# AIM-Harvard/pyradiomics

Measured on AMD Instinct MI355X. Metric: Mvoxels/s for GLCM+GLRLM build, 512^3 vol @32 bins, higher is better.
Workload: dtype u8 levels / u32 counts / f64 out; 1 GPU; GLCM+GLRLM matrix build, 512^3 int32+uint8 volume resident in HBM, 32 grey levels, full mask, 13 angles, uniform levels; one volume per GPU (batch sharding, no collective); size=512, levels=32, dist=uniform, deferred_mode=pipeline

## Files before the change

pyradiomics_amd/csrc/kernels_sweepfw.h:

```cpp
#pragma once
#include "kernels_sweep.h"

namespace prad {

enum FwPhase { FP_INIT, FP_GRAB, FP_CTRL, FP_ISSUE, FP_WAIT_ROWS, FP_WAIT_PACK, FP_GROUP, FP_PACK, FP_SLOW, FP_FLUSH, FP_DRAIN,
               FP_TOTAL, FP_REALTIME, FP_NGROUP, FP_NGROUP_PACK, FP_NSLOW, FP_COUNT };
#ifdef PRAD_FW_STAMPS
__device__ unsigned long long prad_fw_stamps[2 * 8192 * FP_COUNT];
struct FwClock {
  unsigned long long last, first, rt0;
  unsigned acc[FP_COUNT];
  __device__ __forceinline__ void start() {
#pragma unroll
    for (int i = 0; i < FP_COUNT; i++) acc[i] = 0;
    rt0 = __builtin_amdgcn_s_memrealtime();
    first = last = __builtin_readcyclecounter();
  }
  template <int PH>
  __device__ __forceinline__ void lap() {
    const unsigned long long now = __builtin_readcyclecounter();
    acc[PH] += (unsigned)(now - last);
    last = now;
  }
  template <int PH>
// ... 711 lines not shown
              t += U;
              row += U * du;
              off += (long long)U * delta;
              ri += (long long)U * dri;
              zpos += U;
            };
            for (int gi = 0; gi < ng; gi++) {
              load_group(va, off);
              one_group(va, gi == 0);
            }
            if (du != 0 && (row < 0 || row >= NU)) wrap = true;
            continue;
          }
        }
        u32 c[KW];
        if (closing) {
#pragma unroll
          for (int w = 0; w < KW; w++) c[w] = 0;
        } else {
          load_row(lp + off, c);
        }
        clk.template lap<FP_CTRL>();
        single_step(c, tail);
        clk.template lap<FP_SLOW>();
        clk.template count<FP_NSLOW>();
        safe = 0;
        young = 0;
        if (closing) {
          if (finish) break;
          reset_lines(0);
          row -= du * NU;
          off -= (long long)du * NU * D.sU;
          ri -= (long long)du * NU * sUr;
          zpos = 65;
          wrap = false;
          continue;
        }
        t++;
        zpos++;
        row += du;
        off += delta;
        ri += dri;
        if (du != 0 && (row < 0 || row >= NU)) wrap = true;
      }
    }
  }
};

template <bool ZA>
__device__ __forceinline__ void fw_row_word(const FwTab &T, u32 one, int &s, u32 c, u32 x) {
  int t;
#define PRAD_FW_RCOL(J)                                                                                          \
  "v_cmpx_ne_u32_sdwa vcc, %[c], %[x] src0_sel:BYTE_" #J " src1_sel:BYTE_" #J "\n\t"                             \
  "v_add_u32_sdwa %[t], %[s], %[c] dst_sel:DWORD dst_unused:UNUSED_PAD src0_sel:DWORD src1_sel:BYTE_" #J "\n\t"   \
  "v_mul_u32_u24_sdwa %[s], %[P4], %[c] dst_sel:DWORD dst_unused:UNUSED_PAD src0_sel:DWORD src1_sel:BYTE_" #J "\n\t" \
  "v_cmpx_ne_u32_sdwa vcc, %[x], %[z] src0_sel:BYTE_" #J " src1_sel:DWORD\n\t"                                  \
  "ds_add_u32 %[t], %[one]\n\t"                                                                                  \
  "s_mov_b64 exec, -1\n\t"                                                                                       \
  "v_add_u32 %[s], %[Q], %[s]\n\t"
#define PRAD_FW_RCOL_NZ(J)                                                                                       \
  "v_cmpx_ne_u32_sdwa vcc, %[c], %[x] src0_sel:BYTE_" #J " src1_sel:BYTE_" #J "\n\t"                             \
  "v_add_u32_sdwa %[t], %[s], %[c] dst_sel:DWORD dst_unused:UNUSED_PAD src0_sel:DWORD src1_sel:BYTE_" #J "\n\t"   \
  "ds_add_u32 %[t], %[one]\n\t"                                                                                  \
  "v_mul_u32_u24_sdwa %[s], %[P4], %[c] dst_sel:DWORD dst_unused:UNUSED_PAD src0_sel:DWORD src1_sel:BYTE_" #J "\n\t" \
  "s_mov_b64 exec, -1\n\t"                                                                                       \
  "v_add_u32 %[s], %[Q], %[s]\n\t"
  if (ZA) {
    u32 z = 0;
    asm volatile("" : "+v"(z));
    asm volatile(PRAD_FW_RCOL(0) PRAD_FW_RCOL(1) PRAD_FW_RCOL(2) PRAD_FW_RCOL(3)
                 : [s] "+v"(s), [t] "=&v"(t)
                 : [c] "v"(c), [x] "v"(x), [one] "v"(one), [P4] "s"(T.P4), [Q] "s"(T.Q), [z] "v"(z)
                 : "vcc", "memory");
  } else {
    asm volatile(PRAD_FW_RCOL_NZ(0) PRAD_FW_RCOL_NZ(1) PRAD_FW_RCOL_NZ(2) PRAD_FW_RCOL_NZ(3)
                 : [s] "+v"(s), [t] "=&v"(t)
                 : [c] "v"(c), [x] "v"(x), [one] "v"(one), [P4] "s"(T.P4), [Q] "s"(T.Q)
                 : "vcc", "memory");
  }
#undef PRAD_FW_RCOL
#undef PRAD_FW_RCOL_NZ
}

template <bool LONG, bool ZA>
__device__ __forceinline__ void fw_rows_role(const HistLayout &h, const FwTab &T, u32 *lds, const uint8_t *__restrict__ L,
                                             long long nrows, int NX, int pitch, int bx, int nblocks) {
  const int lane = threadIdx.x & 63, wave = threadIdx.x >> 6, wpb = blockDim.x >> 6;
  const int dummy = T.dummy0b + 4 * lane;
  u32 one = 1;
  asm volatile("" : "+v"(one));
  uint8_t *tile = reinterpret_cast<uint8_t *>(lds) + ((fw_lds_bytes(h) + 15) & ~(size_t)15) + (size_t)wave * 64 * PRAD_ROW_PITCH;
  const int RSTEP = nrows >= 4096 ? 8 : 1;
  const long long ngroups = RSTEP == 8 ? ((nrows + 511) / 512) * 8 : (nrows + 63) / 64;
  const long long nwaves = (long long)nblocks * wpb;
  const bool vec16 = (pitch & 15) == 0 && ((uintptr_t)L & 15) == 0;
  for (long long grp = (long long)bx * wpb + wave; grp < ngroups; grp += nwaves) {
    const long long r0 = RSTEP == 8 ? (grp >> 3) * 512 + (grp & 7) : grp * 64;
    int s = 0;
    u32 pw = 0;
    uint4 nx4[4];
    auto fetch = [&](int xc) __attribute__((always_inline)) {
#pragma unroll
      for (int j = 0; j < 4; j++) {
        const int rr = j * 16 + (lane >> 2);
        const int cx = xc + (lane & 3) * 16;
        uint4 q = make_uint4(0, 0, 0, 0);
        if (r0 + RSTEP * rr < nrows && cx < NX) {
          q = *reinterpret_cast<const uint4 *>(L + (r0 + RSTEP * rr) * pitch + cx);
          const int valid = NX - cx;
          if (valid < 16) {
            u32 *qw = reinterpret_cast<u32 *>(&q);
#pragma unroll
            for (int wd = 0; wd < 4; wd++) {
              const int keep = valid - 4 * wd;
              qw[wd] = keep >= 4 ? qw[wd] : (keep <= 0 ? 0u : (qw[wd] & ((1u << (8 * keep)) - 1u)));
            }
          }
        }
        nx4[j] = q;
      }
    };
    if (vec16) fetch(0);
    for (int xc = 0; xc < NX; xc += 64) {
      if (vec16) {
#pragma unroll
        for (int j = 0; j < 4; j++) *reinterpret_cast<uint4 *>(tile + (j * 16 + (lane >> 2)) * PRAD_ROW_PITCH + (lane & 3) * 16) = nx4[j];
        __builtin_amdgcn_wave_barrier();
        if (xc + 64 < NX) fetch(xc + 64);
      } else {
        const bool xin = xc + lane < NX;
#pragma unroll 8
        for (int rr = 0; rr < 64; rr++) {
          uint8_t b = 0;
          if (xin && r0 + RSTEP * rr < nrows) b = L[(r0 + RSTEP * rr) * pitch + xc + lane];
          tile[rr * PRAD_ROW_PITCH + lane] = b;
        }
      }
      __builtin_amdgcn_wave_barrier();
      const uint4 *row = reinterpret_cast<const uint4 *>(tile + lane * PRAD_ROW_PITCH);
#pragma unroll
      for (int q = 0; q < 4; q++) {
        const uint4 d = row[q];
        const u32 wds[4] = {d.x, d.y, d.z, d.w};
        const unsigned m = (pw >> 24) ? (unsigned)(s - __mul24((int)(pw >> 24), T.P4)) : 0u;
        if (LONG && __ballot(m + 16 * T.Q > (unsigned)T.lenlim) != 0) {
#pragma unroll 1
          for (int k = 0; k < 4; k++) {
            const u32 c = wds[k], x = __builtin_amdgcn_alignbyte(c, pw, 3);
            const unsigned m4 = (pw >> 24) ? (unsigned)(s - __mul24((int)(pw >> 24), T.P4)) : 0u;
            if (__ballot(m4 + 4 * T.Q > (unsigned)T.lenlim) != 0) {
#pragma unroll
              for (int b = 0; b < 4; b++) fw_checked<LONG>(T, dummy, s, (int)((x >> (8 * b)) & 0xffu), (int)((c >> (8 * b)) & 0xffu), false);
            } else {
              fw_row_word<ZA>(T, one, s, c, x);
            }
            pw = c;
          }
        } else {
#pragma unroll
          for (int k = 0; k < 4; k++) {
            fw_row_word<ZA>(T, one, s, wds[k], __builtin_amdgcn_alignbyte(wds[k], pw, 3));
            pw = wds[k];
          }
        }
      }
      __builtin_amdgcn_wave_barrier();
    }
    fw_checked<LONG>(T, dummy, s, (int)(pw >> 24), 0, false);
  }
}

template <bool LONG>
__global__ void __launch_bounds__(1024) sweep_fw_rows_kernel(const uint8_t *__restrict__ L, long long nrows, int NX, int pitch,
                                                            int slot, int Ng, int Nr, int RS, u32 *__restrict__ glcm_acc,
                                                            u32 *__restrict__ glrlm_acc, int *__restrict__ flags) {
  extern __shared__ u32 lds[];
  if (flags[0]) return;
  const HistLayout h = hist_layout(true, true, true, Ng, RS);
  if ((unsigned)(size_t)((lds_u32 *)lds) != 0u) {
    if (threadIdx.x == 0) atomicExch(flags + 2, 1);
    return;
  }
  for (int i = threadIdx.x; i < h.words + Ng + 1; i += blockDim.x) lds[i] = 0;
  __syncthreads();
  FwTab T;
  T.init(h, Nr, glrlm_acc + (size_t)slot * Ng * Nr);
  if (flags[3] != 0) fw_rows_role<LONG, true>(h, T, lds, L, nrows, NX, pitch, (int)blockIdx.x, (int)gridDim.x);
  else fw_rows_role<LONG, false>(h, T, lds, L, nrows, NX, pitch, (int)blockIdx.x, (int)gridDim.x);
  flush_block_hist<true, true, true>(lds + Ng + 1, h, Nr, slot, glcm_acc, glrlm_acc);
}

template <bool LONG, int K, bool HASPAD, bool PACK>
__global__ void __launch_bounds__(1024) sweep_fw_kernel(FwSet set, PackJob pj, const uint8_t *__restrict__ L,
                                                        const uint8_t *__restrict__ rowzero, int Ng, int Nr, int RS,
                                                        u32 *__restrict__ glcm_acc, u32 *__restrict__ glrlm_acc,
                                                        int *__restrict__ work, int *__restrict__ flags) {
  extern __shared__ u32 lds[];
  int role = 0;
  while (role + 1 < set.count && (int)blockIdx.x >= set.first_block[role + 1]) role++;
  const int bx = (int)blockIdx.x - set.first_block[role], nblocks = set.first_block[role + 1] - set.first_block[role];
  const int wpb = (int)(blockDim.x >> 6);
  const long long pw = __builtin_amdgcn_readfirstlane((int)(blockIdx.x * wpb + (threadIdx.x >> 6)));
  PackWave pk(pj, pw, (long long)gridDim.x * wpb);
  FwClock clk;
  clk.start();
#ifdef PRAD_FW_SETPRIO
  __builtin_amdgcn_s_setprio(PRAD_FW_SETPRIO);
#endif
  if (flags[0] == 0) {
    const bool anyzero = flags[3] != 0;
    const HistLayout h = hist_layout(true, true, true, Ng, RS);
    if ((unsigned)(size_t)((lds_u32 *)lds) != 0u) {
      if (threadIdx.x == 0) atomicExch(flags + 2, 1);
    } else {
      for (int i = threadIdx.x; i < h.words + Ng + 1; i += blockDim.x) lds[i] = 0;
      __syncthreads();
      clk.lap<FP_INIT>();
      const FwDesc &D = set.d[role];
      FwTab T;
      T.init(h, Nr, glrlm_acc + (size_t)D.slot * Ng * Nr);
      int *wk = work + PRAD_FW_WORK_STRIDE * PRAD_FW_DOMAINS * role;
      if (D.dx == 0) {
        FwWave<LONG, K, 0, HASPAD, PACK> w(T, set.NX);
        w.run(D, set.NX, set.pitch, set.nrows, L, rowzero, anyzero, wk, bx, nblocks, pk, pj, set.xcd != 0, clk);
      } else if (D.dx > 0) {
        FwWave<LONG, K, 1, HASPAD, PACK> w(T, set.NX);
        w.run(D, set.NX, set.pitch, set.nrows, L, rowzero, anyzero, wk, bx, nblocks, pk, pj, set.xcd != 0, clk);
      } else {
        FwWave<LONG, K, -1, HASPAD, PACK> w(T, set.NX);
        w.run(D, set.NX, set.pitch, set.nrows, L, rowzero, anyzero, wk, bx, nblocks, pk, pj, set.xcd != 0, clk);
      }
      clk.lap<FP_CTRL>();
      flush_block_hist<true, true, true>(lds + Ng + 1, h, Nr, D.slot, glcm_acc, glrlm_acc);
      clk.lap<FP_FLUSH>();
    }
  }
  if (PACK) pk.drain(pj);
  clk.lap<FP_DRAIN>();
  clk.store(PACK ? 1 : 0);
}

}
```

pyradiomics_amd/csrc/prad_api.hip:

```cpp
#include "prad_runtime.h"
#include "kernels_generic.h"
#include "kernels_pairs.h"
#include "kernels_sweep.h"
#include "kernels_sweepfw.h"
#include "kernels_sweepfw2.h"
#include "kernels_neigh.h"
#include "kernels_glszm.h"
#include "kernels_voxel.h"
#include "kernels_voxslide.h"
#include "kernels_mcc.h"
#include "kernels_voxtex.h"
#include "kernels_binning.h"

#include <algorithm>
#include <atomic>
#include <chrono>
#include <cmath>
#include <condition_variable>
#include <cstdlib>
#include <deque>
#include <limits>
#include <mutex>
#include <thread>

// ... 140 lines not shown

int generic_glcm(Call &k, int Ng, double *out) {
  const size_t per = (size_t)Ng * Ng * k.Na;
  PRAD_HIP(hipMemsetAsync(out, 0, sizeof(double) * per * k.vm.nvox, k.s));
  const long long threads = (long long)k.vm.nvox * k.vm.boxmax;
  PRAD_TRY(check_grid(threads, "GLCM"));
  Timed t(*k.c, "generic", k.s);
  hipLaunchKernelGGL(gen_glcm_kernel, dim3(blocks_for(threads)), dim3(256), 0, k.s, k.g, k.vm, k.image, k.mask,
                     k.angles_d, k.Na, Ng, out, k.flags_d + 1);
  return check_launch("gen_glcm_kernel");
}

int generic_glrlm(Call &k, int Ng, int Nr, double *out) {
  const size_t per = (size_t)Ng * Nr * k.Na;
  PRAD_HIP(hipMemsetAsync(out, 0, sizeof(double) * per * k.vm.nvox, k.s));
  int *multi = nullptr;
  PRAD_TRY(k.c->get<int>("multi", (size_t)k.vm.nvox * k.Na, &multi));
  PRAD_HIP(hipMemsetAsync(multi, 0, sizeof(int) * k.vm.nvox * k.Na, k.s));
  const long long threads = (long long)k.vm.nvox * k.vm.boxmax * k.Na;
  PRAD_TRY(check_grid(threads, "GLRLM"));
  Timed t(*k.c, "generic", k.s);
  hipLaunchKernelGGL(gen_glrlm_kernel, dim3(blocks_for(threads)), dim3(256), 0, k.s, k.g, k.vm, k.image, k.mask,
                     k.angles_d, k.Na, Ng, Nr, out, multi, k.flags_d + 1);
  PRAD_TRY(check_launch("gen_glrlm_kernel"));
  const long long pthreads = (long long)k.vm.nvox * Ng * k.Na;
  hipLaunchKernelGGL(glrlm_prune_kernel, dim3(blocks_for(pthreads)), dim3(256), 0, k.s, out, multi, k.vm.nvox, Ng,
                     Nr, k.Na);
  return check_launch("glrlm_prune_kernel");
}

int generic_gldm(Call &k, int Ng, int alpha, double *out) {
  const size_t per = (size_t)Ng * (2 * (size_t)k.Na + 1);
  PRAD_HIP(hipMemsetAsync(out, 0, sizeof(double) * per * k.vm.nvox, k.s));
  const long long threads = (long long)k.vm.nvox * k.vm.boxmax;
  PRAD_TRY(check_grid(threads, "GLDM"));
  Timed t(*k.c, "generic", k.s);
  hipLaunchKernelGGL(gen_gldm_kernel, dim3(blocks_for(threads)), dim3(256), 0, k.s, k.g, k.vm, k.image, k.mask,
                     k.angles_d, k.Na, Ng, alpha, out, k.flags_d + 1);
  return check_launch("gen_gldm_kernel");
}

int generic_ngtdm(Call &k, int Ng, double *out) {
  Timed t(*k.c, "generic", k.s);
  if (k.vm.voxels) {
    hipLaunchKernelGGL(gen_ngtdm_voxel_kernel, dim3(blocks_for(k.vm.nvox, 64)), dim3(64), 0, k.s, k.g, k.vm,
                       k.image, k.mask, k.angles_d, k.Na, Ng, out, k.flags_d + 1);
    return check_launch("gen_ngtdm_voxel_kernel");
  }
  unsigned long long *acc = nullptr;
  const size_t nacc = (size_t)Ng * (k.Na + 1);
  PRAD_TRY(k.c->get<unsigned long long>("ngtdm_acc", nacc, &acc));
  PRAD_HIP(hipMemsetAsync(acc, 0, sizeof(unsigned long long) * nacc, k.s));
  PRAD_TRY(check_grid(k.g.n, "NGTDM"));
  hipLaunchKernelGGL(gen_ngtdm_segment_kernel, dim3(blocks_for(k.g.n)), dim3(256), 0, k.s, k.g, k.vm, k.image,
                     k.mask, k.angles_d, k.Na, Ng, acc, k.flags_d + 1);
  PRAD_TRY(check_launch("gen_ngtdm_segment_kernel"));
  hipLaunchKernelGGL(ngtdm_finalize_kernel, dim3(blocks_for(Ng, 64)), dim3(64), 0, k.s, acc, Ng, k.Na, out);
  return check_launch("ngtdm_finalize_kernel");
}

struct SweepPlan {
  bool ok = false;
  int Nz = 1, Ny = 1, Nx = 1;
  SweepSet lines;
  int row_slot = -1;
  bool skip1 = false;
  bool fused = false;
  int LPL = 1;
  int pitch = 0, padw = 0;
  bool vec_rows = false;
  AngleSet aset;
  int RS = 0;
  bool LONG = false;
  int threads = 256;
  size_t lds_bytes = 0;
  int RSr = 0;
  bool LONGr = false;
  size_t lds_bytes_rows = 0;
  bool fw = false;
  int fwK = 8;
  int fw_blocks = 1;
  int fw_threads = 1024;
  int fw_rows_threads = 512;
  int RSfw = 0;
  bool LONGfw = false;
  size_t lds_fw = 0;
  int RSfw_rows = 0;
  size_t lds_fw_rows = 0;
  bool fw2 = false;
  int RS2 = 0;
  int fw2_copies = 1;
  bool LONGfw2 = false;
  size_t lds_fw2 = 0;
  int pitch16 = 0;
  bool fw2_rows = false;
  int RS2r = 0, fw2r_copies = 1, fw2r_waves = 16;
  bool LONGfw2r = false;
  size_t lds_fw2_rows = 0;
  FwSet fwset;
};

constexpr size_t kHistBudget = 72 * 1024;
constexpr size_t kHistBudgetRows = 36 * 1024;
constexpr int kRowsThreads = 512;
constexpr size_t kHistBudgetFw = 146 * 1024;

int cu_count() {
  static thread_local int cus = 0;
  if (!cus) {
    int dev = 0;
    if (hipGetDevice(&dev) != hipSuccess ||
        hipDeviceGetAttribute(&cus, hipDeviceAttributeMultiprocessorCount, dev) != hipSuccess || cus <= 0)
      cus = 256;
  }
  return cus;
}

int fit_rs(bool glcm, bool glrlm, bool fused, int Ng, int Nr, size_t budget) {
  int lo = 0, hi = Nr;
  if (sizeof(u32) * (size_t)hist_layout(glcm, glrlm, fused, Ng, 1).words > budget) return -1;
  lo = 1;
  while (lo < hi) {
    const int mid = (lo + hi + 1) / 2;
    if (sizeof(u32) * (size_t)hist_layout(glcm, glrlm, fused, Ng, mid).words <= budget) lo = mid;
    else hi = mid - 1;
  }
  return lo;
}

SweepPlan plan_sweep(const Call &k, int Ng, int Nr, bool want_glcm, bool want_glrlm) {
  SweepPlan p;
  if (k.vm.voxels || k.g.nd > 3 || Ng < 1 || Ng > 255 || k.Na > PRAD_MAX_SWEEP) return p;
  int dims[3] = {1, 1, 1};
  for (int d = 0; d < k.g.nd; d++) dims[3 - k.g.nd + d] = k.g.size[d];
  p.Nz = dims[0]; p.Ny = dims[1]; p.Nx = dims[2];
  const int longest = std::max(dims[0], std::max(dims[1], dims[2]));
  if (want_glrlm && Nr < longest) return p;
  if (!want_glrlm) Nr = 1;
  if (want_glcm && want_glrlm) {
    const int rs = fit_rs(true, true, true, Ng, Nr, kHistBudget);
    const int rsr = fit_rs(true, true, true, Ng, Nr, kHistBudgetRows);
    if (Ng <= (255 >> PRAD_FUSED_SHIFT) && rs >= std::min(Nr, 8) && rsr >= std::min(Nr, 4)) {
      p.fused = true;
      p.RS = rs;
      p.RSr = rsr;
    }
  }
  const bool force_fw2 = getenv("PRAD_FORCE_FW2") != nullptr && Ng >= 8;
  if (force_fw2 && want_glcm && want_glrlm && p.Nx > 64 && p.Nx <= 512) p.fused = false;
  if (want_glcm && want_glrlm && !p.fused && (Ng >= 40 || force_fw2) && p.Nx > 64 && p.Nx <= 512 && !getenv("PRAD_NO_FW2")) {
    const long long maxwords = (158 * 1024) / 4;
    const long long room = maxwords / (Ng + 1) - (Ng + 1);
    int copies = 1;
    long long rs2 = std::min<long long>(room, Nr);
    for (int cc = 8; cc >= 2; cc >>= 1)
      if (room / cc >= std::min<long long>(32, Nr)) {
        copies = cc;
        rs2 = std::min<long long>(std::min<long long>(room / cc, 64), Nr);
        break;
      }
    if (const char *e = getenv("PRAD_FW2_COPIES")) {
      copies = std::max(1, std::min(8, atoi(e)));
      rs2 = std::min<long long>(std::min<long long>(room / copies, copies > 1 ? 64 : Nr), Nr);
    }
    if (const char *e = getenv("PRAD_FW2_RS")) rs2 = std::min<long long>(rs2, atoll(e));
    if (rs2 < Nr && ((Ng + 1 + copies * rs2) & 1) == 0) rs2--;
// ... 46 lines not shown
  if (const char *e = getenv("PRAD_THREADS")) {
    const int v = atoi(e);
    if (v == 256 || v == 512 || v == 1024) p.threads = v;
  }
  const size_t hw = (size_t)hist_layout(want_glcm, want_glrlm, p.fused, Ng, p.RSr).words;
  p.lds_bytes_rows = sizeof(u32) * ((hw + 3) & ~(size_t)3) + (kRowsThreads / 64) * 64 * PRAD_ROW_PITCH;
  {
    const double waves = std::max(1.0, (double)(cu_count() / std::max(1, std::min(k.Na, 12))) * 16.0);
    const double cost[3] = {1.0, 0.575, 0.33};
    const int cand[3] = {4, 2, 1};
    double best = 1e300;
    p.LPL = 1;
    for (int i = 0; i < 3; i++) {
      if (cand[i] > 1 && p.Nx < 48 * cand[i]) continue;
      const double chunks = (double)std::max(p.Ny, 1) * ((p.Nx + 64 * cand[i] - 1) / (64 * cand[i]));
      const double t = (chunks <= waves ? 1.0 : chunks / waves + 0.5) * cost[i];
      if (t < best) {
        best = t;
        p.LPL = cand[i];
      }
    }
  }
  if (const char *e = getenv("PRAD_LPL")) {
    const int v = atoi(e);
    if (v == 1 || v == 2 || v == 4) p.LPL = v;
  }
  p.vec_rows = (p.Nx % 16) == 0;
  p.fw = p.fused && p.Nx > 64 && p.Nx <= 1024 && !getenv("PRAD_NO_FW");
  if (p.Nx > 512 && getenv("PRAD_NO_FW16")) p.fw = false;
  if (const char *e = getenv("PRAD_FW_MINVOX")) p.fw = p.fw && k.g.n >= atoll(e);
  p.fwK = p.Nx <= 256 ? 4 : (p.Nx <= 512 ? 8 : 16);
  if (p.fw2) p.fwK = p.Nx <= 256 ? 4 : 8;
  p.padw = (p.fw || p.fw2) ? 0 : std::min(64 * p.LPL, p.Nx);
  p.pitch16 = 2 * ((p.Nx + 7) & ~7);
  p.pitch = (p.Nx + p.padw + 15) & ~15;
  p.lines.count = 0;
  p.aset.count = k.Na;
  for (int a = 0; a < k.Na; a++) {
    int o[3] = {0, 0, 0};
    for (int d = 0; d < k.g.nd; d++) o[3 - k.g.nd + d] = k.angles_h[a * k.g.nd + d];
    int first = 0;
    for (int d = 0; d < 3; d++) {
      if (o[d] < -1 || o[d] > 1) return p;
      if (!first && o[d]) first = o[d];
      p.aset.off[a][d] = o[d];
    }
    if (first != 1) return p;
    if (o[0] == 0 && o[1] == 0) {
      if (p.row_slot >= 0) return p;
      p.row_slot = a;
      continue;
    }
    SweepDesc &D = p.lines.d[p.lines.count++];
    D.slot = a;
    D.NX = p.Nx;
    D.dx = o[2];
    if (o[0] == 1) {
      D.NM = p.Nz; D.NU = p.Ny; D.du = o[1];
      D.sM = (long long)p.Ny * p.pitch; D.sU = p.pitch;
    } else {
      D.NM = p.Ny; D.NU = p.Nz; D.du = 0;
      D.sM = p.pitch; D.sU = (long long)p.Ny * p.pitch;
    }
    D.LXc = (p.Nx + 64 * p.LPL - 1) / (64 * p.LPL);
    D.chunks = (long long)D.NU * D.LXc;
  }
  if ((p.fw || p.fw2) && p.lines.count > 0) {
    size_t budget = kHistBudgetFw;
    if (const char *e = getenv("PRAD_FW_BUDGET_KB")) budget = (size_t)std::max(8, atoi(e)) * 1024;
    p.RSfw = fit_rs(true, true, true, Ng, Nr, budget);
    if (p.RSfw < Nr) {
      for (int rs = p.RSfw; rs >= std::max(16, p.RSfw - 12); rs--) {
        const int d = (((rs + 1) * (Ng + 1)) % 32 + 1) % 32, dist = std::min(d, 32 - d);
        if ((d & 1) && dist >= 5 && dist <= 11) {
          p.RSfw = rs;
          break;
        }
      }
    }
    if (const char *e = getenv("PRAD_FW_RS")) p.RSfw = std::max(1, std::min(p.RSfw, atoi(e)));
    p.LONGfw = p.RSfw < Nr;
    p.lds_fw = fw_lds_bytes(hist_layout(true, true, true, Ng, p.RSfw));
    if (p.row_slot >= 0 && p.fw) {
      if (const char *e = getenv("PRAD_FW_ROWS_THREADS")) p.fw_rows_threads = std::max(64, std::min(1024, atoi(e) & ~63));
      const size_t tiles = (size_t)(p.fw_rows_threads / 64) * 64 * PRAD_ROW_PITCH;
      int rs = fit_rs(true, true, true, Ng, Nr, std::min<size_t>(100 * 1024, (size_t)160 * 1024 - 2048 - tiles));
      for (int r = rs; rs < Nr && r >= std::max(16, rs - 12); r--) {
        const int d = (((r + 1) * (Ng + 1)) % 32 + 1) % 32, dist = std::min(d, 32 - d);
        if ((d & 1) && dist >= 5 && dist <= 11) { rs = r; break; }
      }
      p.RSfw_rows = rs;
      p.lds_fw_rows = ((fw_lds_bytes(hist_layout(true, true, true, Ng, rs)) + 15) & ~(size_t)15) + tiles;
    }
    {
      const int nroles = p.lines.count;
      int total = cu_count();
      if (const char *e = getenv("PRAD_FW_BLOCKS")) total = std::max(nroles, atoi(e));
      if (const char *e = getenv("PRAD_FW_THREADS")) p.fw_threads = std::max(64, std::min(1024, atoi(e) & ~63));
      int bonus[PRAD_MAX_SWEEP] = {0};
      {
        int left = total % nroles;
        const bool as_listed = getenv("PRAD_FW_EXTRA_FIRST") != nullptr;
        for (int cls = as_listed ? 0 : 2; cls >= 0 && left > 0; cls--)
          for (int r = 0; r < nroles && left > 0; r++) {
            const SweepDesc &S = p.lines.d[r];
            const int c = (S.dx != 0 ? 1 : 0) + (S.du != 0 ? 1 : 0);
            if ((as_listed || c == cls) && !bonus[r]) {
              bonus[r] = 1;
              left--;
            }
          }
      }
      p.fwset.first_block[0] = 0;
      for (int r = 0; r < nroles; r++) p.fwset.first_block[r + 1] = p.fwset.first_block[r] + total / nroles + bonus[r];
      for (int r = nroles + 1; r < PRAD_MAX_SWEEP + 1; r++) p.fwset.first_block[r] = p.fwset.first_block[nroles];
      p.fw_blocks = p.fwset.first_block[nroles];
    }
    int per_wave = 6;
    if (const char *e = getenv("PRAD_FW_PER_WAVE")) per_wave = std::max(1, atoi(e));
    p.fwset.count = p.lines.count;
    p.fwset.NX = p.Nx;
    p.fwset.xcd = 0;
    if (const char *e = getenv("PRAD_FW_XCD")) p.fwset.xcd = ((p.fw || p.fw2) && p.Nz >= 64 && atoi(e) != 0) ? 1 : 0;
    for (int i = 0; i < p.lines.count; i++) {
      const SweepDesc &S = p.lines.d[i];
      FwDesc &D = p.fwset.d[i];
      D.slot = S.slot; D.NM = S.NM; D.NU = S.NU; D.du = S.du; D.dx = S.dx; D.sM = S.sM; D.sU = S.sU;
      p.fwset.pitch = p.pitch;
      if (p.fw2) {
        const bool march_z = S.sM >= S.sU;
        D.sM = march_z ? (long long)p.Ny * p.pitch16 : p.pitch16;
        D.sU = march_z ? p.pitch16 : (long long)p.Ny * p.pitch16;
        p.fwset.pitch = p.pitch16;
      }
      p.fwset.nrows = p.Nz * p.Ny;
      const long long want = (long long)per_wave * (p.fwset.first_block[i + 1] - p.fwset.first_block[i]) * (p.fw_threads / 64);
      int pieces = (int)std::max<long long>(1, (want + D.NU - 1) / D.NU);
      int CL = ((D.NM + pieces - 1) / pieces + 7) & ~7;
      CL = std::max(CL, D.NM >= 128 ? 64 : 16);
      const bool march_z_role = S.sM >= S.sU && p.Nz > 1;
      D.dom_kind = march_z_role ? 0 : 1;
      if (p.fwset.xcd && march_z_role) CL = std::max(32, ((D.NM + PRAD_FW_DOMAINS - 1) / PRAD_FW_DOMAINS + 7) & ~7);
      if (const char *e = getenv("PRAD_FW_CL")) CL = std::max(8, atoi(e) & ~7);
      D.CL = CL;
      D.pieces = (D.NM + CL - 1) / CL;
      const long long chunks = (long long)D.NU * D.pieces;
      if (chunks > 2000000000LL) return p;
      D.chunks = (int)chunks;
    }
  } else {
    p.fw = false;
    if (p.fw2) return SweepPlan();
  }
  if (p.row_slot < 0) p.skip1 = false;
  p.ok = true;
  return p;
}

template <bool G, bool R, bool LNG, bool F, int LPL>
int launch_lines_lpl(Call &k, const SweepPlan &p, const uint8_t *levels, int Ng, int Nr, u32 *glcm_acc,
                     u32 *glrlm_acc, int *multi) {
  long long maxchunks = 0;
  for (int i = 0; i < p.lines.count; i++) maxchunks = std::max(maxchunks, p.lines.d[i].chunks);
  const int wpb = p.threads / 64;
  const long long blocks_avail = std::max<long long>(1, (long long)cu_count() / p.lines.count);
  unsigned gx = (unsigned)std::max<long long>(1, std::min<long long>(blocks_avail, (maxchunks + wpb - 1) / wpb));
  if (const char *e = getenv("PRAD_LINES_BLOCKS")) {
    const int v = atoi(e);
// ... 4 lines not shown
  hipLaunchKernelGGL((sweep_lines_kernel<G, R, LNG, F, LPL>), dim3(gx, p.lines.count), dim3(p.threads), p.lds_bytes,
                     k.s, p.lines, levels, Ng, Nr, p.RS, glcm_acc, glrlm_acc, multi, multi + PRAD_MAX_SWEEP,
                     k.flags_d);
  return check_launch("sweep_lines_kernel");
}

template <bool G, bool R, bool LNG, bool F>
int launch_lines(Call &k, const SweepPlan &p, const uint8_t *levels, int Ng, int Nr, u32 *glcm_acc, u32 *glrlm_acc,
                 int *multi) {
  if (p.LPL == 4) return launch_lines_lpl<G, R, LNG, F, 4>(k, p, levels, Ng, Nr, glcm_acc, glrlm_acc, multi);
  if (p.LPL == 2) return launch_lines_lpl<G, R, LNG, F, 2>(k, p, levels, Ng, Nr, glcm_acc, glrlm_acc, multi);
  return launch_lines_lpl<G, R, LNG, F, 1>(k, p, levels, Ng, Nr, glcm_acc, glrlm_acc, multi);
}

template <bool LNG, int K, bool HASPAD, bool PACK>
int launch_fw_kpp(Call &k, const SweepPlan &p, const PackJob &pj, const uint8_t *levels, const uint8_t *rowzero, int Ng, int Nr,
                  u32 *glcm_acc, u32 *glrlm_acc, int *multi, int *flags_d) {
  PRAD_HIP(hipFuncSetAttribute(reinterpret_cast<const void *>(&sweep_fw_kernel<LNG, K, HASPAD, PACK>),
                               hipFuncAttributeMaxDynamicSharedMemorySize, (int)p.lds_fw));
  hipLaunchKernelGGL((sweep_fw_kernel<LNG, K, HASPAD, PACK>), dim3(p.fw_blocks), dim3(p.fw_threads), p.lds_fw, k.s, p.fwset, pj,
                     levels, rowzero, Ng, Nr, p.RSfw, glcm_acc, glrlm_acc, multi + 2 * PRAD_MAX_SWEEP + PRAD_FW_WORK_STRIDE, flags_d);
  return check_launch("sweep_fw_kernel");
}
template <bool LNG, int K, bool HASPAD>
int launch_fw_kp(Call &k, const SweepPlan &p, const PackJob &pj, const uint8_t *levels, const uint8_t *rowzero, int Ng, int Nr,
                 u32 *glcm_acc, u32 *glrlm_acc, int *multi, int *flags_d) {
  if (pj.n16 > 0) return launch_fw_kpp<LNG, K, HASPAD, true>(k, p, pj, levels, rowzero, Ng, Nr, glcm_acc, glrlm_acc, multi, flags_d);
  return launch_fw_kpp<LNG, K, HASPAD, false>(k, p, pj, levels, rowzero, Ng, Nr, glcm_acc, glrlm_acc, multi, flags_d);
}
template <bool LNG, int K>
int launch_fw_k(Call &k, const SweepPlan &p, const PackJob &pj, const uint8_t *levels, const uint8_t *rowzero, int Ng, int Nr,
                u32 *glcm_acc, u32 *glrlm_acc, int *multi, int *flags_d) {
  if (p.Nx != 64 * K) return launch_fw_kp<LNG, K, true>(k, p, pj, levels, rowzero, Ng, Nr, glcm_acc, glrlm_acc, multi, flags_d);
  return launch_fw_kp<LNG, K, false>(k, p, pj, levels, rowzero, Ng, Nr, glcm_acc, glrlm_acc, multi, flags_d);
}
int launch_fw(Call &k, const SweepPlan &p, const PackJob &pj, const uint8_t *levels, const uint8_t *rowzero, int Ng, int Nr,
              u32 *glcm_acc, u32 *glrlm_acc, int *multi, int *flags_d) {
  if (p.fwK == 16)
    return p.LONGfw ? launch_fw_k<true, 16>(k, p, pj, levels, rowzero, Ng, Nr, glcm_acc, glrlm_acc, multi, flags_d)
                    : launch_fw_k<false, 16>(k, p, pj, levels, rowzero, Ng, Nr, glcm_acc, glrlm_acc, multi, flags_d);
  if (p.LONGfw) return p.fwK == 4 ? launch_fw_k<true, 4>(k, p, pj, levels, rowzero, Ng, Nr, glcm_acc, glrlm_acc, multi, flags_d)
                                : launch_fw_k<true, 8>(k, p, pj, levels, rowzero, Ng, Nr, glcm_acc, glrlm_acc, multi, flags_d);
  return p.fwK == 4 ? launch_fw_k<false, 4>(k, p, pj, levels, rowzero, Ng, Nr, glcm_acc, glrlm_acc, multi, flags_d)
                    : launch_fw_k<false, 8>(k, p, pj, levels, rowzero, Ng, Nr, glcm_acc, glrlm_acc, multi, flags_d);
}

template <bool LNG, int K, bool HASPAD, bool SKIP1, bool PACK>
int launch_fw2_khsp(Call &k, const SweepPlan &p, const PackJob &pj, const uint8_t *levels16, int Ng, int Nr, u32 *glcm_acc, u32 *glrlm_acc,
                    int *work, int *flags_d) {
  PRAD_HIP(hipFuncSetAttribute(reinterpret_cast<const void *>(&sweep_fw2_kernel<LNG, K, HASPAD, SKIP1, PACK>),
                               hipFuncAttributeMaxDynamicSharedMemorySize, (int)p.lds_fw2));
  hipLaunchKernelGGL((sweep_fw2_kernel<LNG, K, HASPAD, SKIP1, PACK>), dim3(p.fw_blocks), dim3(1024), p.lds_fw2, k.s, p.fwset, pj, levels16,
                     Ng, Nr, p.RS2, p.fw2_copies, glcm_acc, glrlm_acc, work, flags_d);
  return check_launch("sweep_fw2_kernel");
}
template <bool LNG, int K, bool HASPAD, bool SKIP1>
int launch_fw2_khs(Call &k, const SweepPlan &p, const PackJob &pj, const uint8_t *levels16, int Ng, int Nr, u32 *glcm_acc, u32 *glrlm_acc,
                   int *work, int *flags_d) {
  if (pj.n16 > 0) return launch_fw2_khsp<LNG, K, HASPAD, SKIP1, true>(k, p, pj, levels16, Ng, Nr, glcm_acc, glrlm_acc, work, flags_d);
  return launch_fw2_khsp<LNG, K, HASPAD, SKIP1, false>(k, p, pj, levels16, Ng, Nr, glcm_acc, glrlm_acc, work, flags_d);
}
template <bool LNG, int K>
int launch_fw2_k(Call &k, const SweepPlan &p, const PackJob &pj, const uint8_t *levels16, int Ng, int Nr, u32 *glcm_acc, u32 *glrlm_acc,
                 int *multi, int *flags_d) {
  int *work = multi + 2 * PRAD_MAX_SWEEP + PRAD_FW_WORK_STRIDE;
  if (p.Nx != 64 * K)
    return p.skip1 ? launch_fw2_khs<LNG, K, true, true>(k, p, pj, levels16, Ng, Nr, glcm_acc, glrlm_acc, work, flags_d)
                   : launch_fw2_khs<LNG, K, true, false>(k, p, pj, levels16, Ng, Nr, glcm_acc, glrlm_acc, work, flags_d);
  return p.skip1 ? launch_fw2_khs<LNG, K, false, true>(k, p, pj, levels16, Ng, Nr, glcm_acc, glrlm_acc, work, flags_d)
                 : launch_fw2_khs<LNG, K, false, false>(k, p, pj, levels16, Ng, Nr, glcm_acc, glrlm_acc, work, flags_d);
}
int launch_fw2(Call &k, const SweepPlan &p, const PackJob &pj, const uint8_t *levels16, int Ng, int Nr, u32 *glcm_acc, u32 *glrlm_acc,
               int *multi, int *flags_d) {
  if (p.LONGfw2) return p.fwK == 4 ? launch_fw2_k<true, 4>(k, p, pj, levels16, Ng, Nr, glcm_acc, glrlm_acc, multi, flags_d)
                                 : launch_fw2_k<true, 8>(k, p, pj, levels16, Ng, Nr, glcm_acc, glrlm_acc, multi, flags_d);
  return p.fwK == 4 ? launch_fw2_k<false, 4>(k, p, pj, levels16, Ng, Nr, glcm_acc, glrlm_acc, multi, flags_d)
                    : launch_fw2_k<false, 8>(k, p, pj, levels16, Ng, Nr, glcm_acc, glrlm_acc, multi, flags_d);
}

template <bool LNG>
int launch_fw_rows(Call &k, const SweepPlan &p, const uint8_t *levels, int Ng, int Nr, u32 *glcm_acc, u32 *glrlm_acc, int *flags_d) {
  const long long nrows = (long long)p.Nz * p.Ny, groups = nrows >= 4096 ? ((nrows + 511) / 512) * 8 : (nrows + 63) / 64;
  const int wpb = p.fw_rows_threads / 64;
  const unsigned gx = (unsigned)std::max<long long>(1, std::min<long long>((groups + wpb - 1) / wpb, (long long)cu_count()));
  PRAD_HIP(hipFuncSetAttribute(reinterpret_cast<const void *>(&sweep_fw_rows_kernel<LNG>),
                               hipFuncAttributeMaxDynamicSharedMemorySize, (int)p.lds_fw_rows));
  hipLaunchKernelGGL((sweep_fw_rows_kernel<LNG>), dim3(gx), dim3(p.fw_rows_threads), p.lds_fw_rows, k.s, levels, nrows, p.Nx,
                     p.pitch, p.row_slot, Ng, Nr, p.RSfw_rows, glcm_acc, glrlm_acc, flags_d);
  return check_launch("sweep_fw_rows_kernel");
}

template <bool LNG>
int launch_fw2_rows(Call &k, const SweepPlan &p, const uint8_t *levels16, int Ng, int Nr, u32 *glcm_acc, u32 *glrlm_acc, int *flags_d) {
  const long long nrows = (long long)p.Nz * p.Ny, groups = nrows >= 4096 ? ((nrows + 511) / 512) * 8 : (nrows + 63) / 64;
  const int wpb = p.fw2r_waves;
  const unsigned gx = (unsigned)std::max<long long>(1, std::min<long long>((groups + wpb - 1) / wpb, (long long)cu_count()));
  PRAD_HIP(hipFuncSetAttribute(reinterpret_cast<const void *>(&sweep_fw2_rows_kernel<LNG>),
                               hipFuncAttributeMaxDynamicSharedMemorySize, (int)p.lds_fw2_rows));
  hipLaunchKernelGGL((sweep_fw2_rows_kernel<LNG>), dim3(gx), dim3(64 * wpb), p.lds_fw2_rows, k.s, levels16, nrows, p.Nx, p.pitch16,
                     p.row_slot, Ng, Nr, p.RS2r, p.fw2r_copies, glcm_acc, glrlm_acc, flags_d);
  return check_launch("sweep_fw2_rows_kernel");
}

template <bool G, bool R, bool LNG, bool F>
int launch_rows(Call &k, const SweepPlan &p, const uint8_t *levels, int Ng, int Nr, u32 *glcm_acc, u32 *glrlm_acc,
                int *multi) {
  const long long nrows = (long long)p.Nz * p.Ny;
  const long long groups = (nrows + 63) / 64;
  const int wpb = kRowsThreads / 64;
  const int per_cu = std::max(1, std::min(2048 / kRowsThreads, (int)(160 * 1024 / p.lds_bytes_rows)));
  const unsigned gx = (unsigned)std::max<long long>(1, std::min<long long>((groups + wpb - 1) / wpb, (long long)cu_count() * per_cu));
  PRAD_HIP(hipFuncSetAttribute(reinterpret_cast<const void *>(&sweep_rows_kernel<G, R, LNG, F>),
                               hipFuncAttributeMaxDynamicSharedMemorySize, (int)p.lds_bytes_rows));
  hipLaunchKernelGGL((sweep_rows_kernel<G, R, LNG, F>), dim3(gx), dim3(kRowsThreads), p.lds_bytes_rows, k.s, levels,
                     nrows, p.Nx, p.pitch, p.row_slot, Ng, Nr, p.RSr, glcm_acc, glrlm_acc, multi, k.flags_d);
  return check_launch("sweep_rows_kernel");
}

__global__ void __launch_bounds__(256) zero3_kernel(u32 *__restrict__ a, size_t na, u32 *__restrict__ b, size_t nb,
                                                    u32 *__restrict__ c3, size_t nc) {
  const size_t t = (size_t)blockIdx.x * blockDim.x + threadIdx.x, nt = (size_t)gridDim.x * blockDim.x;
  uint4 *a4 = reinterpret_cast<uint4 *>(a);
  for (size_t i = t; i < na / 4; i += nt) a4[i] = make_uint4(0, 0, 0, 0);
  for (size_t i = (na & ~(size_t)3) + t; i < na; i += nt) a[i] = 0;
  for (size_t i = t; i < nb; i += nt) b[i] = 0;
  for (size_t i = t; i < nc; i += nt) c3[i] = 0;
}

struct VolState {
  bool valid = false;
  SweepPlan p;
  int Ng = 0, Nr = 0, Na = 0;
  double *glcm = nullptr, *glrlm = nullptr;
  uint8_t *levels = nullptr, *rowzero = nullptr;
  uint8_t *levels16 = nullptr;
  u32 *acc = nullptr, *glcm_acc = nullptr, *glrlm_acc = nullptr;
  int *multi = nullptr;
  int *flags_d = nullptr;
  bool packed_inline = false;
  int lane = -1;
};

bool fin_side() {
  static const bool on = getenv("PRAD_FINALIZE_STREAM") != nullptr && atoi(getenv("PRAD_FINALIZE_STREAM")) != 0;
  return on;
}
int fin_wait_for_lane(hipStream_t s, int lane);

int vol_prepare(Call &k, const SweepPlan &p, int Ng, int Nr, double *glcm, double *glrlm, VolState &v) {
  Context &c = *k.c;
  if (fin_side() && c.lane >= 0) PRAD_TRY(fin_wait_for_lane(k.s, c.lane));
  v.lane = c.lane;
  v.valid = true;
  v.p = p;
  v.Ng = Ng;
  v.Nr = Nr;
  v.Na = k.Na;
  v.glcm = glcm;
  v.glrlm = glrlm;
  v.flags_d = k.flags_d;
  const long long nrows = (long long)p.Nz * p.Ny;
  v.levels = nullptr;
  if (!(p.fw2 && p.fw2_rows && p.lines.count > 0 && p.row_slot >= 0) || getenv("PRAD_FW2_KEEP8")) {
    PRAD_TRY(c.get<uint8_t>("levels", (size_t)nrows * p.pitch + 1024, &v.levels));
    v.levels += 512;
  }
  v.levels16 = nullptr;
  if (p.fw2) {
    PRAD_TRY(c.get<uint8_t>("levels16", (size_t)nrows * p.pitch16 + 4096, &v.levels16));
    v.levels16 += 2048;
  }
// ... 1820 lines not shown
```

Measured before the change: 287,500 Mvoxels/s.

## Double-buffer fw rows tile in 32-column halves and overlap loads with LDS zeroing

```diff
diff --git a/pyradiomics_amd/csrc/kernels_sweepfw.h b/pyradiomics_amd/csrc/kernels_sweepfw.h
--- a/pyradiomics_amd/csrc/kernels_sweepfw.h
+++ b/pyradiomics_amd/csrc/kernels_sweepfw.h
@@ -817,65 +817,88 @@
 #undef PRAD_FW_RCOL_NZ
 }
 
+#define PRAD_FW_ROW_PITCH 48
+
 template <bool LONG, bool ZA>
 __device__ __forceinline__ void fw_rows_role(const HistLayout &h, const FwTab &T, u32 *lds, const uint8_t *__restrict__ L,
-                                             long long nrows, int NX, int pitch, int bx, int nblocks) {
+                                             long long nrows, int NX, int pitch, int bx, int nblocks, int Ng, bool novec) {
   const int lane = threadIdx.x & 63, wave = threadIdx.x >> 6, wpb = blockDim.x >> 6;
   const int dummy = T.dummy0b + 4 * lane;
   u32 one = 1;
   asm volatile("" : "+v"(one));
-  uint8_t *tile = reinterpret_cast<uint8_t *>(lds) + ((fw_lds_bytes(h) + 15) & ~(size_t)15) + (size_t)wave * 64 * PRAD_ROW_PITCH;
+  uint8_t *tile = reinterpret_cast<uint8_t *>(lds) + ((fw_lds_bytes(h) + 15) & ~(size_t)15) + (size_t)wave * 64 * PRAD_FW_ROW_PITCH;
   const int RSTEP = nrows >= 4096 ? 8 : 1;
   const long long ngroups = RSTEP == 8 ? ((nrows + 511) / 512) * 8 : (nrows + 63) / 64;
   const long long nwaves = (long long)nblocks * wpb;
-  const bool vec16 = (pitch & 15) == 0 && ((uintptr_t)L & 15) == 0;
-  for (long long grp = (long long)bx * wpb + wave; grp < ngroups; grp += nwaves) {
-    const long long r0 = RSTEP == 8 ? (grp >> 3) * 512 + (grp & 7) : grp * 64;
+  const bool vec16 = (pitch & 15) == 0 && ((uintptr_t)L & 15) == 0 && !novec;
+  long long r0 = 0;
+  uint4 nx4[4];
+  auto fetch = [&](int xc) __attribute__((always_inline)) {
+#pragma unroll
+    for (int j = 0; j < 4; j++) {
+      const int rr = j * 16 + (lane >> 2);
+      const int cx = xc + (lane & 3) * 16;
+      uint4 q = make_uint4(0, 0, 0, 0);
+      if (r0 + RSTEP * rr < nrows && cx < NX) {
+        q = *reinterpret_cast<const uint4 *>(L + (r0 + RSTEP * rr) * pitch + cx);
+        const int valid = NX - cx;
+        if (valid < 16) {
+          u32 *qw = reinterpret_cast<u32 *>(&q);
+#pragma unroll
+          for (int wd = 0; wd < 4; wd++) {
+            const int keep = valid - 4 * wd;
+            qw[wd] = keep >= 4 ? qw[wd] : (keep <= 0 ? 0u : (qw[wd] & ((1u << (8 * keep)) - 1u)));
+          }
+        }
+      }
+      nx4[j] = q;
+    }
+  };
+  auto stage = [&](int hx) __attribute__((always_inline)) {
+    if (vec16) {
+      if (((lane >> 1) & 1) == ((hx >> 5) & 1)) {
+#pragma unroll
+        for (int j = 0; j < 4; j++) *reinterpret_cast<uint4 *>(tile + (j * 16 + (lane >> 2)) * PRAD_FW_ROW_PITCH + (lane & 1) * 16) = nx4[j];
+      }
+    } else {
+      const bool xin = hx + (lane & 31) < NX;
+#pragma unroll 8
+      for (int rr = lane >> 5; rr < 64; rr += 2) {
+        uint8_t b = 0;
+        if (xin && r0 + RSTEP * rr < nrows) b = L[(r0 + RSTEP * rr) * pitch + hx + (lane & 31)];
+        tile[rr * PRAD_FW_ROW_PITCH + (lane & 31)] = b;
+      }
+    }
+  };
+  const uint4 *row = reinterpret_cast<const uint4 *>(tile + lane * PRAD_FW_ROW_PITCH);
+  long long grp = (long long)bx * wpb + wave;
+  if (grp < ngroups) {
+    r0 = RSTEP == 8 ? (grp >> 3) * 512 + (grp & 7) : grp * 64;
+    if (vec16) fetch(0);
+  }
+  for (int i = threadIdx.x; i < h.words + Ng + 1; i += blockDim.x) lds[i] = 0;
+  __syncthreads();
+  for (; grp < ngroups; grp += nwaves) {
     int s = 0;
     u32 pw = 0;
-    uint4 nx4[4];
-    auto fetch = [&](int xc) __attribute__((always_inline)) {
-#pragma unroll
-      for (int j = 0; j < 4; j++) {
-        const int rr = j * 16 + (lane >> 2);
-        const int cx = xc + (lane & 3) * 16;
-        uint4 q = make_uint4(0, 0, 0, 0);
-        if (r0 + RSTEP * rr < nrows && cx < NX) {
-          q = *reinterpret_cast<const uint4 *>(L + (r0 + RSTEP * rr) * pitch + cx);
-          const int valid = NX - cx;
-          if (valid < 16) {
-            u32 *qw = reinterpret_cast<u32 *>(&q);
-#pragma unroll
-            for (int wd = 0; wd < 4; wd++) {
-              const int keep = valid - 4 * wd;
-              qw[wd] = keep >= 4 ? qw[wd] : (keep <= 0 ? 0u : (qw[wd] & ((1u << (8 * keep)) - 1u)));
-            }
-          }
-        }
-        nx4[j] = q;
-      }
-    };
-    if (vec16) fetch(0);
-    for (int xc = 0; xc < NX; xc += 64) {
-      if (vec16) {
-#pragma unroll
-        for (int j = 0; j < 4; j++) *reinterpret_cast<uint4 *>(tile + (j * 16 + (lane >> 2)) * PRAD_ROW_PITCH + (lane & 3) * 16) = nx4[j];
+    uint4 cur[2], nxt[2];
+    stage(0);
+    __builtin_amdgcn_wave_barrier();
+    cur[0] = row[0];
+    cur[1] = row[1];
+    nxt[0] = nxt[1] = make_uint4(0, 0, 0, 0);
+    for (int hx = 0; hx < NX; hx += 32) {
+      __builtin_amdgcn_wave_barrier();
+      if (hx + 32 < NX) {
+        stage(hx + 32);
         __builtin_amdgcn_wave_barrier();
-        if (xc + 64 < NX) fetch(xc + 64);
-      } else {
-        const bool xin = xc + lane < NX;
-#pragma unroll 8
-        for (int rr = 0; rr < 64; rr++) {
-          uint8_t b = 0;
-          if (xin && r0 + RSTEP * rr < nrows) b = L[(r0 + RSTEP * rr) * pitch + xc + lane];
-          tile[rr * PRAD_ROW_PITCH + lane] = b;
-        }
-      }
-      __builtin_amdgcn_wave_barrier();
-      const uint4 *row = reinterpret_cast<const uint4 *>(tile + lane * PRAD_ROW_PITCH);
-#pragma unroll
-      for (int q = 0; q < 4; q++) {
-        const uint4 d = row[q];
+        if (vec16 && (hx & 32) == 0 && hx + 64 < NX) fetch(hx + 64);
+        nxt[0] = row[0];
+        nxt[1] = row[1];
+      }
+#pragma unroll
+      for (int q = 0; q < 2; q++) {
+        const uint4 d = cur[q];
         const u32 wds[4] = {d.x, d.y, d.z, d.w};
         const unsigned m = (pw >> 24) ? (unsigned)(s - __mul24((int)(pw >> 24), T.P4)) : 0u;
         if (LONG && __ballot(m + 16 * T.Q > (unsigned)T.lenlim) != 0) {
@@ -899,16 +922,22 @@
           }
         }
       }
-      __builtin_amdgcn_wave_barrier();
+      cur[0] = nxt[0];
+      cur[1] = nxt[1];
     }
     fw_checked<LONG>(T, dummy, s, (int)(pw >> 24), 0, false);
+    if (grp + nwaves < ngroups) {
+      const long long g2 = grp + nwaves;
+      r0 = RSTEP == 8 ? (g2 >> 3) * 512 + (g2 & 7) : g2 * 64;
+      if (vec16) fetch(0);
+    }
   }
 }
 
 template <bool LONG>
 __global__ void __launch_bounds__(1024) sweep_fw_rows_kernel(const uint8_t *__restrict__ L, long long nrows, int NX, int pitch,
                                                             int slot, int Ng, int Nr, int RS, u32 *__restrict__ glcm_acc,
-                                                            u32 *__restrict__ glrlm_acc, int *__restrict__ flags) {
+                                                            u32 *__restrict__ glrlm_acc, int *__restrict__ flags, int novec) {
   extern __shared__ u32 lds[];
   if (flags[0]) return;
   const HistLayout h = hist_layout(true, true, true, Ng, RS);
@@ -916,12 +945,10 @@
     if (threadIdx.x == 0) atomicExch(flags + 2, 1);
     return;
   }
-  for (int i = threadIdx.x; i < h.words + Ng + 1; i += blockDim.x) lds[i] = 0;
-  __syncthreads();
   FwTab T;
   T.init(h, Nr, glrlm_acc + (size_t)slot * Ng * Nr);
-  if (flags[3] != 0) fw_rows_role<LONG, true>(h, T, lds, L, nrows, NX, pitch, (int)blockIdx.x, (int)gridDim.x);
-  else fw_rows_role<LONG, false>(h, T, lds, L, nrows, NX, pitch, (int)blockIdx.x, (int)gridDim.x);
+  if (flags[3] != 0) fw_rows_role<LONG, true>(h, T, lds, L, nrows, NX, pitch, (int)blockIdx.x, (int)gridDim.x, Ng, novec != 0);
+  else fw_rows_role<LONG, false>(h, T, lds, L, nrows, NX, pitch, (int)blockIdx.x, (int)gridDim.x, Ng, novec != 0);
   flush_block_hist<true, true, true>(lds + Ng + 1, h, Nr, slot, glcm_acc, glrlm_acc);
 }
 
diff --git a/pyradiomics_amd/csrc/prad_api.hip b/pyradiomics_amd/csrc/prad_api.hip
--- a/pyradiomics_amd/csrc/prad_api.hip
+++ b/pyradiomics_amd/csrc/prad_api.hip
@@ -246,6 +246,8 @@
   int fw_blocks = 1;
   int fw_threads = 1024;
   int fw_rows_threads = 512;
+  int fw_rows_blocks = 0;
+  bool fw_rows_novec = false;
   int RSfw = 0;
   bool LONGfw = false;
   size_t lds_fw = 0;
@@ -458,8 +460,12 @@
     p.LONGfw = p.RSfw < Nr;
     p.lds_fw = fw_lds_bytes(hist_layout(true, true, true, Ng, p.RSfw));
     if (p.row_slot >= 0 && p.fw) {
+      const long long nrows = (long long)p.Nz * p.Ny, groups = nrows >= 4096 ? ((nrows + 511) / 512) * 8 : (nrows + 63) / 64;
+      p.fw_rows_threads = groups > 8LL * cu_count() ? 1024 : 512;
       if (const char *e = getenv("PRAD_FW_ROWS_THREADS")) p.fw_rows_threads = std::max(64, std::min(1024, atoi(e) & ~63));
-      const size_t tiles = (size_t)(p.fw_rows_threads / 64) * 64 * PRAD_ROW_PITCH;
+      if (const char *e = getenv("PRAD_FW_ROWS_BLOCKS")) p.fw_rows_blocks = std::max(0, atoi(e));
+      p.fw_rows_novec = getenv("PRAD_FW_ROWS_NOVEC") != nullptr;
+      const size_t tiles = (size_t)(p.fw_rows_threads / 64) * 64 * PRAD_FW_ROW_PITCH;
       int rs = fit_rs(true, true, true, Ng, Nr, std::min<size_t>(100 * 1024, (size_t)160 * 1024 - 2048 - tiles));
       for (int r = rs; rs < Nr && r >= std::max(16, rs - 12); r--) {
         const int d = (((r + 1) * (Ng + 1)) % 32 + 1) % 32, dist = std::min(d, 32 - d);
@@ -630,11 +636,11 @@
 int launch_fw_rows(Call &k, const SweepPlan &p, const uint8_t *levels, int Ng, int Nr, u32 *glcm_acc, u32 *glrlm_acc, int *flags_d) {
   const long long nrows = (long long)p.Nz * p.Ny, groups = nrows >= 4096 ? ((nrows + 511) / 512) * 8 : (nrows + 63) / 64;
   const int wpb = p.fw_rows_threads / 64;
-  const unsigned gx = (unsigned)std::max<long long>(1, std::min<long long>((groups + wpb - 1) / wpb, (long long)cu_count()));
+  const unsigned gx = (unsigned)std::max<long long>(1, std::min<long long>((groups + wpb - 1) / wpb, (long long)(p.fw_rows_blocks > 0 ? p.fw_rows_blocks : cu_count())));
   PRAD_HIP(hipFuncSetAttribute(reinterpret_cast<const void *>(&sweep_fw_rows_kernel<LNG>),
                                hipFuncAttributeMaxDynamicSharedMemorySize, (int)p.lds_fw_rows));
   hipLaunchKernelGGL((sweep_fw_rows_kernel<LNG>), dim3(gx), dim3(p.fw_rows_threads), p.lds_fw_rows, k.s, levels, nrows, p.Nx,
-                     p.pitch, p.row_slot, Ng, Nr, p.RSfw_rows, glcm_acc, glrlm_acc, flags_d);
+                     p.pitch, p.row_slot, Ng, Nr, p.RSfw_rows, glcm_acc, glrlm_acc, flags_d, p.fw_rows_novec ? 1 : 0);
   return check_launch("sweep_fw_rows_kernel");
 }
 
```

New measurement: 286,800 Mvoxels/s. Within noise of the previous version (-0.3%).
